# SajayR/TRIAD

Measured on AMD Instinct MI355X. Metric: tri-modal triples/sec (whole node) + loss parity, B=256 at 1/2/4/8 MI355X, higher is better.
Workload: dtype bf16

## Files before the change

include/triad_hip.h:

```cpp
#ifndef TRIAD_HIP_H
#define TRIAD_HIP_H

#include <hip/hip_runtime_api.h>

#ifdef __cplusplus
extern "C" {
#endif

#define TRIAD_EINVAL 1001

int triad_pairsim_nparts(int R_pad, int Bk);

int triad_pairsim_fwd(const void* Q, const void* K, int R, int R_pad, int Nq, int Bq, int Bk, int Nk_pad,
                      int Nk_eff, int D, const float* temp, float clamp_lo, int diag, int diag_off,
                      float* rowmax, int* argmax, double* nn_part, float* diagS, void* dS, long long CT,
                      double* st_part, const int* k_len, hipStream_t stream);

typedef struct triad_pairsim_problem {
  const void* Q;
  const void* K;
  int R, R_pad, Nq, Bq, Bk, Nk_pad, Nk_eff;
  const float* temp;
  float clamp_lo;
  int diag, diag_off;
// ... 128 lines not shown
                       hipStream_t stream);

int triad_grad_sumsq(const float* g, const void* chunks, int nchunks, double* out, hipStream_t stream);
int triad_adamw_step(float* p, const float* g, float* m, float* v, const void* chunks, int nchunks,
                     const float* pp, const float* scale, float beta1, float beta2, float omb1, float omb2,
                     float eps, const unsigned long long* shadow, hipStream_t stream);
int triad_gather_grads(const void* pieces, int npieces, float* g, int accumulate, hipStream_t stream);

int triad_gather_rows(const void* src, long long src_rows, const int* idx, int B, int M, int row_bytes, void* dst,
                      hipStream_t stream);

int triad_l2norm_rows(const void* x, int rows, int D, float eps, void* y, hipStream_t stream);

int triad_retrieval_maxmean_f32(const float* Q, const int* qlen, int Bq, int nq_pad, const float* K, const int* klen,
                                int Bk, int nk_pad, int D, float temp, float* sim, hipStream_t stream);

int triad_l2norm_rows_f32(const float* x, int rows, int D, float eps, float* y, hipStream_t stream);

long long triad_chgn_workspace_bytes(int B, int T, int C);
int triad_chgn_gelu_fwd(const void* x, int B, int T, int Tp, int C, const float* gamma, const float* beta,
                        float eps, float* mean, float* rstd, void* ws, void* y, hipStream_t stream);
int triad_chgn_gelu_bwd(const void* x, const void* dy, int B, int T, int Tp, int C, const float* gamma,
                        const float* beta, const float* mean, const float* rstd, void* ws, void* dx, float* dgamma,
                        float* dbeta, hipStream_t stream);

int triad_c0gn_fwd(const void* wave, long long Lp, const void* w0, int B, int T, int Tp, int C, const float* gamma,
                   const float* beta, float eps, float* mean, float* rstd, void* ws, void* out, void* y0out,
                   hipStream_t stream);

long long triad_conv0_dw_workspace_bytes(int B, int T, int C);
int triad_conv0_dw(const void* wave, long long Lp, const void* dy0, int B, int T, int Tp, int C, void* ws, float* dw0,
                   hipStream_t stream);

int triad_posconv(const void* x, const void* wt, const float* bias, void* y, int B, int T, int C, int groups,
                  int pad, hipStream_t stream);

long long triad_posconv_dw_part_bytes(int C, int groups, int splits);
int triad_posconv_dw(const void* x, const void* dy, int B, int T, int C, int groups, int pad, int splits, float* part,
                     hipStream_t stream);

int triad_attn_fwd(const void* q, long long q_sB, long long q_sN, const void* k, long long k_sB, long long k_sN,
                   const void* v, long long v_sB, long long v_sN, int B, int H, int N, int D, float scale, void* out,
                   long long out_sB, long long out_sN, float* lse, hipStream_t stream);
int triad_attn_bwd(const void* q, long long q_sB, long long q_sN, const void* k, long long k_sB, long long k_sN,
                   const void* v, long long v_sB, long long v_sN, const void* o, long long o_sB, long long o_sN,
                   const void* dout, long long do_sB, long long do_sN, const float* lse, int B, int H, int N, int D,
                   float scale, void* dq, long long dq_sB, long long dq_sN, void* dk, long long dk_sB,
                   long long dk_sN, void* dv, long long dv_sB, long long dv_sN, float* delta, hipStream_t stream);
int triad_attn_dropmask(int B, int H, int N, float p, unsigned seed, unsigned* wq, unsigned* wk, hipStream_t stream);
int triad_attn_fwd_dropout(const void* q, long long q_sB, long long q_sN, const void* k, long long k_sB,
                           long long k_sN, const void* v, long long v_sB, long long v_sN, int B, int H, int N, int D,
                           float scale, const unsigned* wq, float p, void* out, long long out_sB, long long out_sN,
                           float* lse, hipStream_t stream);
int triad_attn_bwd_dropout(const void* q, long long q_sB, long long q_sN, const void* k, long long k_sB,
                           long long k_sN, const void* v, long long v_sB, long long v_sN, const void* o,
                           long long o_sB, long long o_sN, const void* dout, long long do_sB, long long do_sN,
                           const float* lse, int B, int H, int N, int D, float scale, const unsigned* wq,
                           const unsigned* wk, float p, void* dq, long long dq_sB, long long dq_sN, void* dk,
                           long long dk_sB, long long dk_sN, void* dv, long long dv_sB, long long dv_sN, float* delta,
                           hipStream_t stream);

int triad_attn_long_dropmask(int B, int H, int N, float p, unsigned seed, unsigned* wq, unsigned* wk,
                             hipStream_t stream);
int triad_attn_long_fwd(const void* q, long long q_sB, long long q_sN, const void* k, long long k_sB, long long k_sN,
                        const void* v, long long v_sB, long long v_sN, int B, int H, int N, int D, float scale,
                        const unsigned* wq, float p, void* out, long long out_sB, long long out_sN, float* lse,
                        hipStream_t stream);
int triad_attn_long_bwd(const void* q, long long q_sB, long long q_sN, const void* k, long long k_sB, long long k_sN,
                        const void* v, long long v_sB, long long v_sN, const void* o, long long o_sB, long long o_sN,
                        const void* dout, long long do_sB, long long do_sN, const float* lse, int B, int H, int N,
                        int D, float scale, const unsigned* wq, const unsigned* wk, float p, void* dq, long long dq_sB,
                        long long dq_sN, void* dk, long long dk_sB, long long dk_sN, void* dv, long long dv_sB,
// ... 44 lines not shown
```

triad_amd/_lib.py:

```python
from __future__ import annotations

import ctypes as C
import os
import threading

_HERE = os.path.dirname(os.path.abspath(__file__))
DEFAULT_LIB = os.path.join(_HERE, "libtriad_hip.so")
LIB_PATH = os.environ.get("TRIAD_LIB_VARIANT", DEFAULT_LIB)

vp, i32, u32, i64, f32, f64 = C.c_void_p, C.c_int, C.c_uint, C.c_longlong, C.c_float, C.c_double

SIGNATURES = {
    "triad_pairsim_nparts": [i32, i32],
    "triad_pairsim_fwd": [vp, vp, i32, i32, i32, i32, i32, i32, i32, i32, vp, f32, i32, i32, vp, vp, vp, vp, vp,
                          i64, vp, vp, vp],
    "triad_pairsim_fwd_multi": [vp, i32, vp],
    "triad_pairsim_diag": [vp, i32, vp],
    "triad_clip_reduce": [vp, i32, i32, i32, i32, vp, vp, vp, vp],
    "triad_diag_smooth": [vp, i32, i32, i32, i32, f64, vp, vp, vp, vp],
    "triad_diag_sparsity": [vp, i32, i32, i32, i32, f32, f64, vp, vp, vp, vp],
    "triad_losshead": [vp, i32, i32, vp, vp, i32, f64, vp, i32, f64, f32, vp, vp, vp, vp],
    "triad_pairsim_dS": [vp, vp, i32, i32, i32, i32, i32, i32, i32, i32, vp, f32, i32, i32, vp, vp, vp, vp, vp,
                         vp, i64, vp, vp],
    "triad_split_pack": [vp, i32, i32, i32, i64, vp, vp, vp],
# ... 16 lines not shown
    "triad_gemm_bf16_bias_bf16": [vp, i64, i32, vp, i64, i32, i32, i32, i32, vp, vp, i64, vp],
    "triad_gemm_bf16_splitk": [vp, i64, i32, vp, i64, i32, i32, i32, i32, i32, vp, vp, vp, i32, vp],
    "triad_gemm_bf16_splitk_form": [vp, i64, i32, vp, i64, i32, i32, i32, i32, i32, vp, vp, vp, i32, i32, vp],
    "triad_wpack": [vp, i32, vp, vp],
    "triad_wpack2": [vp, i32, vp, vp, i32, vp, vp],
    "triad_projhead_fwd": [vp, i64, i32, i64, i64, i64, vp, vp, vp, vp, f32, vp, vp, vp, vp, vp, vp, vp, vp],
    "triad_similarity_maps": [vp, vp, i32, i32, i32, i32, vp, f32, vp, vp],
    "triad_rowpanel_count": [i64],
    "triad_projhead_ln_fwd": [vp, i64, i32, i64, i64, i64, vp, vp, vp, vp, f32, vp, vp, vp, vp, vp],
    "triad_rowgemm_bias": [vp, i64, i32, i64, vp, vp, vp, vp],
    "triad_projhead_ln_bwd": [vp, i64, vp, vp, vp, vp, vp, vp, vp, vp],
    "triad_ln_fwd": [vp, i32, vp, vp, f32, vp, vp, vp, vp],
    "triad_ln_bwd3": [vp, vp, vp, vp, vp, i32, vp, vp, i32, vp],
    "triad_sum_slabs": [vp, i32, i64, vp, i32, vp, vp],
    "triad_colsum_splits": [i64, i32],
    "triad_colsum": [vp, i64, i32, i64, vp, f32, i32, vp, vp],
    "triad_colsum_dma_splits": [i64, i32],
    "triad_colsum_dma": [vp, i64, i32, i64, vp, f32, i32, vp, vp],
    "triad_global_znorm": [vp, i64, f32, vp, vp, i32, vp],
    "triad_grad_sumsq": [vp, vp, i32, vp, vp],
    "triad_adamw_step": [vp, vp, vp, vp, vp, i32, vp, vp, f32, f32, f32, f32, f32, vp, vp],
    "triad_gather_grads": [vp, i32, vp, i32, vp],
    "triad_gather_rows": [vp, i64, vp, i32, i32, i32, vp, vp],
    "triad_l2norm_rows": [vp, i32, i32, f32, vp, vp],
    "triad_l2norm_rows_f32": [vp, i32, i32, f32, vp, vp],
    "triad_retrieval_maxmean_f32": [vp, vp, i32, i32, vp, vp, i32, i32, i32, f32, vp, vp],
    "triad_chgn_workspace_bytes": [i32, i32, i32],
    "triad_chgn_gelu_fwd": [vp, i32, i32, i32, i32, vp, vp, f32, vp, vp, vp, vp, vp],
    "triad_chgn_gelu_bwd": [vp, vp, i32, i32, i32, i32, vp, vp, vp, vp, vp, vp, vp, vp, vp],
    "triad_gemm_bf16_form": [vp, i64, i32, vp, i64, i32, i32, i32, i32, vp, vp, i64, i32, i32, vp],
    "triad_conv0_dw_workspace_bytes": [i32, i32, i32],
    "triad_conv0_dw": [vp, i64, vp, i32, i32, i32, i32, vp, vp, vp],
    "triad_c0gn_fwd": [vp, i64, vp, i32, i32, i32, i32, vp, vp, f32, vp, vp, vp, vp, vp, vp],
    "triad_posconv": [vp, vp, vp, vp, i32, i32, i32, i32, i32, vp],
    "triad_posconv_dw_part_bytes": [i32, i32, i32],
    "triad_posconv_dw": [vp, vp, i32, i32, i32, i32, i32, i32, vp, vp],
    "triad_rows_nt": [vp, i64, i32, i32, vp, i32, vp, vp],
    "triad_lora_update": [vp, i64, i32, i32, vp, vp, vp],
    "triad_dropaddln_fwd": [vp, vp, vp, vp, f32, i32, i32, f32, u32, vp, vp, vp, vp, vp],
    "triad_dropaddln_bwd_blocks": [i32],
    "triad_dropaddln_bwd": [vp, vp, vp, vp, vp, vp, vp, i32, i32, f32, u32, vp, vp, vp, vp],
    "triad_gelu_table_bytes": [],
    "triad_gelu_table": [vp, vp],
    "triad_geludrop_fwd": [vp, i64, f32, u32, vp, vp, vp],
    "triad_geludrop_bwd": [vp, vp, i64, f32, u32, vp, vp, vp],
    "triad_dropout_keep": [i64, f32, u32, vp, vp],
    "triad_addln_fwd": [vp, vp, vp, vp, vp, f32, i32, i32, vp, vp, i32, vp, vp, vp],
    "triad_addln_bwd": [vp, i32, vp, vp, vp, vp, vp, vp, i32, i32, vp, vp, vp],
    "triad_lora_tn_blocks": [i32],
    "triad_lora_tn": [vp, i64, i32, i32, vp, vp, vp, f32, vp, vp, vp],
    "triad_attn_dropmask": [i32, i32, i32, f32, u32, vp, vp, vp],
    "triad_attn_fwd_dropout": [vp, i64, i64, vp, i64, i64, vp, i64, i64, i32, i32, i32, i32, f32, vp, f32, vp, i64,
                               i64, vp, vp],
    "triad_attn_bwd_dropout": [vp, i64, i64, vp, i64, i64, vp, i64, i64, vp, i64, i64, vp, i64, i64, vp, i32, i32,
                               i32, i32, f32, vp, vp, f32, vp, i64, i64, vp, i64, i64, vp, i64, i64, vp, vp],
    "triad_attn_fwd": [vp, i64, i64, vp, i64, i64, vp, i64, i64, i32, i32, i32, i32, f32, vp, i64, i64, vp, vp],
    "triad_attn_bwd": [vp, i64, i64, vp, i64, i64, vp, i64, i64, vp, i64, i64, vp, i64, i64, vp, i32, i32, i32,
                       i32, f32, vp, i64, i64, vp, i64, i64, vp, i64, i64, vp, vp],
    "triad_attn_long_dropmask": [i32, i32, i32, f32, u32, vp, vp, vp],
    "triad_attn_long_fwd": [vp, i64, i64, vp, i64, i64, vp, i64, i64, i32, i32, i32, i32, f32, vp, f32, vp, i64, i64,
                            vp, vp],
    "triad_attn_long_bwd": [vp, i64, i64, vp, i64, i64, vp, i64, i64, vp, i64, i64, vp, i64, i64, vp, i32, i32, i32,
                            i32, f32, vp, vp, f32, vp, i64, i64, vp, i64, i64, vp, i64, i64, vp, vp],
    "triad_dense_nparts": [i64],
    "triad_dense_rowmax": [vp, i32, i32, i32, i32, i32, vp, vp, vp],
    "triad_nonneg_fwd": [vp, i64, f32, vp, vp],
    "triad_nonneg_bwd": [vp, i64, f32, f32, vp, vp, vp],
    "triad_sims_bwd_pack": [vp, vp, vp, vp, vp, i32, i32, i32, i32, i32, vp, vp, i64, vp, vp],
    "triad_sum_parts": [vp, i32, f64, vp, vp],
}
RESTYPES = {"triad_pairsim_nparts": C.c_int, "triad_chgn_workspace_bytes": C.c_longlong,
            "triad_conv0_dw_workspace_bytes": C.c_longlong, "triad_gelu_table_bytes": C.c_longlong,
            "triad_posconv_dw_part_bytes": C.c_longlong,
            "triad_lora_tn_blocks": C.c_int, "triad_dropaddln_bwd_blocks": C.c_int,
            "triad_colsum_splits": C.c_int, "triad_colsum_dma_splits": C.c_int, "triad_dense_nparts": C.c_int,
            "triad_rowpanel_count": C.c_int}

BACKBONE_ENTRY_POINTS = frozenset({
    "triad_chgn_gelu_fwd", "triad_chgn_gelu_bwd", "triad_gemm_bf16_form", "triad_conv0_dw", "triad_c0gn_fwd",
    "triad_posconv", "triad_posconv_dw", "triad_gemm_bf16_splitk", "triad_rows_nt", "triad_lora_update",
    "triad_dropaddln_fwd", "triad_dropaddln_bwd", "triad_gelu_table", "triad_geludrop_fwd", "triad_geludrop_bwd",
    "triad_dropout_keep", "triad_addln_fwd", "triad_addln_bwd", "triad_lora_tn", "triad_attn_dropmask",
    "triad_attn_fwd_dropout", "triad_attn_bwd_dropout", "triad_attn_fwd", "triad_attn_bwd",
    "triad_attn_long_dropmask", "triad_attn_long_fwd", "triad_attn_long_bwd"})


def hot_path_entry_points():
    return tuple(n for n in SIGNATURES if n not in RESTYPES and n not in BACKBONE_ENTRY_POINTS)



class PairsimProblem(C.Structure):
    _fields_ = [("Q", vp), ("K", vp), ("R", i32), ("R_pad", i32), ("Nq", i32), ("Bq", i32), ("Bk", i32),
                ("Nk_pad", i32), ("Nk_eff", i32), ("temp", vp), ("clamp_lo", f32), ("diag", i32), ("diag_off", i32),
                ("rowmax", vp), ("argmax", vp), ("nn_part", vp), ("diagS", vp), ("dS", vp), ("CT", i64),
                ("st_part", vp), ("k_tiles", vp)]


_lock = threading.Lock()
_lib = None


class TriadError(RuntimeError):
    pass


def load():
    global _lib
    with _lock:
        if _lib is None:
            if not os.path.exists(LIB_PATH):
                raise TriadError(f"{LIB_PATH} not found: build it with `python -m triad_amd.build` "
# ... 73 lines not shown
```

triad_amd/csrc/frontend.hip:

```cpp
#include "common.h"

namespace {

constexpr int CHUNK = 128;
constexpr int NT = 256;

struct V8 {
  float v[8];
};

__device__ __forceinline__ V8 load8(const bf16* p) {
  const bf16x8 r = *(const bf16x8*)p;
  V8 o;
#pragma unroll
  for (int i = 0; i < 8; ++i) o.v[i] = (float)r[i];
  return o;
}

__device__ __forceinline__ void store8(bf16* p, const V8& x) {
  bf16x8 r;
#pragma unroll
  for (int i = 0; i < 8; ++i) r[i] = (bf16)x.v[i];
  *(bf16x8*)p = r;
}
// ... 282 lines not shown
  for (int t = t0 + r0; t < t1; t += rows) {
    const V8 dv = load8(dy + ((size_t)b * Tp + t) * C + c0);
    const float* sp = smp + C0_S * (t - t0);
#pragma unroll
    for (int j = 0; j < C0_K; ++j) {
      const float sj = sp[j];
#pragma unroll
      for (int i = 0; i < 8; ++i) dw[i][j] = fmaf(dv.v[i], sj, dw[i][j]);
    }
  }
  float* dst = dwpart + ((size_t)b * nblk + blk) * C * C0_K;
#pragma unroll
  for (int j0 = 0; j0 < C0_K; j0 += 2) {
    __syncthreads();
#pragma unroll
    for (int i = 0; i < 8; ++i) {
      red[(threadIdx.x * 8 + i) * 2] = dw[i][j0];
      red[(threadIdx.x * 8 + i) * 2 + 1] = dw[i][j0 + 1];
    }
    __syncthreads();
    for (int c = threadIdx.x; c < C; c += NT) {
      const int g8 = c / 8, i = c % 8;
      float a0 = 0.f, a1 = 0.f;
      for (int r = 0; r < rows; ++r) {
        a0 += red[((r * tpr + g8) * 8 + i) * 2];
        a1 += red[((r * tpr + g8) * 8 + i) * 2 + 1];
      }
      dst[c * C0_K + j0] = a0;
      dst[c * C0_K + j0 + 1] = a1;
    }
  }
}

bool shape_ok(int B, int T, int C) {
  return B > 0 && T > 0 && C > 0 && C % 8 == 0 && NT % (C / 8) == 0;
}

}

extern "C" {

long long triad_chgn_workspace_bytes(int B, int T, int C) {
  const long long nchunk = (T + CHUNK - 1) / CHUNK;
  return (long long)B * nchunk * C * 8 + (long long)B * C * 8 + (long long)B * C * 16;
}

int triad_chgn_gelu_fwd(const void* x, int B, int T, int Tp, int C, const float* gamma, const float* beta,
                        float eps, float* mean, float* rstd, void* ws, void* y, hipStream_t stream) {
  if (!shape_ok(B, T, C) || Tp < T) return TRIAD_EINVAL;
  const int nchunk = (T + CHUNK - 1) / CHUNK;
  float2* part = (float2*)ws;
  hipLaunchKernelGGL(chgn_sums_kernel<0>, dim3(nchunk, B), dim3(NT), 0, stream, (const bf16*)x, nullptr, T, Tp, C,
                     nullptr, nullptr, nullptr, nullptr, part);
  hipLaunchKernelGGL(chgn_stats_kernel, dim3((C + 255) / 256, B), dim3(256), 0, stream, part, nchunk, T, C, eps,
                     mean, rstd);
  hipLaunchKernelGGL(chgn_apply_kernel<0>, dim3(nchunk, B), dim3(NT), 0, stream, (const bf16*)x, nullptr, T, Tp, C,
                     mean, rstd, gamma, beta, nullptr, (bf16*)y);
  TRIAD_CHECK_LAUNCH();
  return TRIAD_OK;
}

int triad_chgn_gelu_bwd(const void* x, const void* dy, int B, int T, int Tp, int C, const float* gamma,
                        const float* beta, const float* mean, const float* rstd, void* ws, void* dx, float* dgamma,
                        float* dbeta, hipStream_t stream) {
  if (!shape_ok(B, T, C) || Tp < T) return TRIAD_EINVAL;
  const int nchunk = (T + CHUNK - 1) / CHUNK;
// ... 10 lines not shown
  TRIAD_CHECK_LAUNCH();
  return TRIAD_OK;
}

int triad_c0gn_fwd(const void* wave, long long Lp, const void* w0, int B, int T, int Tp, int C, const float* gamma,
                   const float* beta, float eps, float* mean, float* rstd, void* ws, void* out, void* y0out,
                   hipStream_t stream) {
  if (!shape_ok(B, T, C) || Tp < T || Lp < (long long)C0_S * (Tp - 1) + C0_K) return TRIAD_EINVAL;
  const int nchunk = (T + CHUNK - 1) / CHUNK;
  float2* part = (float2*)ws;
  hipLaunchKernelGGL(c0gn_kernel<0>, dim3(nchunk, B), dim3(NT), 0, stream, (const bf16*)wave, Lp, (const bf16*)w0, T,
                     Tp, C, nullptr, nullptr, nullptr, nullptr, nullptr, nullptr, part);
  hipLaunchKernelGGL(chgn_stats_kernel, dim3((C + 255) / 256, B), dim3(256), 0, stream, part, nchunk, T, C, eps,
                     mean, rstd);
  hipLaunchKernelGGL(c0gn_kernel<1>, dim3(nchunk, B), dim3(NT), 0, stream, (const bf16*)wave, Lp, (const bf16*)w0, T,
                     Tp, C, mean, rstd, gamma, beta, (bf16*)out, (bf16*)y0out, nullptr);
  TRIAD_CHECK_LAUNCH();
  return TRIAD_OK;
}

long long triad_conv0_dw_workspace_bytes(int B, int T, int C) {
  return (long long)B * ((T + C0_DW_ROWS - 1) / C0_DW_ROWS) * C * C0_K * 4;
}

int triad_conv0_dw(const void* wave, long long Lp, const void* dy0, int B, int T, int Tp, int C, void* ws, float* dw0,
                   hipStream_t stream) {
  if (!shape_ok(B, T, C) || Tp < T || Lp < (long long)C0_S * (T - 1) + C0_K) return TRIAD_EINVAL;
  const int nblk = (T + C0_DW_ROWS - 1) / C0_DW_ROWS;
  hipLaunchKernelGGL(c0dw_kernel, dim3(nblk, B), dim3(NT), 0, stream, (const bf16*)wave, Lp, (const bf16*)dy0, T, Tp,
                     C, (float*)ws);
  TRIAD_CHECK_LAUNCH();
  return triad_sum_slabs((const float*)ws, B * nblk, (long long)C * C0_K, nullptr, 0, dw0, stream);
}
}
```

triad_amd/frontend.py:

```python
from __future__ import annotations

import types
from ctypes import c_void_p as C_void_p

import torch
import torch.nn as nn
import torch.nn.functional as F

from . import _lib
from ._lib import call, ptr, stream_ptr


def _compute_dtype(x):
    if x.is_cuda and torch.is_autocast_enabled("cuda"):
        return torch.get_autocast_dtype("cuda")
    return x.dtype


class _Conv1dGemm(torch.autograd.Function):

    @staticmethod
    def forward(ctx, x, w, bias, stride, need_dx, cd):
        B, T, C = x.shape
        O, Cw, k = w.shape
# ... 153 lines not shown

class _Conv0GNGelu(torch.autograd.Function):

    @staticmethod
    def forward(ctx, wave, w, gamma, beta, eps, Tp):
        B, L = wave.shape
        O = w.shape[0]
        T = (L - 10) // 5 + 1
        need = (Tp - 1) * 5 + 10
        xw = F.pad(wave.to(torch.bfloat16), (0, max(0, need - L))).contiguous()
        w0 = w.to(torch.bfloat16).reshape(O, 10).contiguous()
        g = gamma.detach().float().contiguous()
        b = beta.detach().float().contiguous()
        dev = wave.device
        mean = torch.empty(B, O, dtype=torch.float32, device=dev)
        rstd = torch.empty(B, O, dtype=torch.float32, device=dev)
        ws = torch.empty(int(call("triad_chgn_workspace_bytes", B, T, O)), dtype=torch.uint8, device=dev)
        out = torch.empty(B * Tp + 2, O, dtype=torch.bfloat16, device=dev)
        y0 = torch.empty(B * Tp, O, dtype=torch.bfloat16, device=dev)
        out[B * Tp:].zero_()
        call("triad_c0gn_fwd", ptr(xw), xw.shape[1], ptr(w0), B, T, Tp, O, ptr(g), ptr(b), float(eps), ptr(mean),
             ptr(rstd), ptr(ws), ptr(out), ptr(y0), stream_ptr(dev))
        ctx.save_for_backward(xw, y0, g, b, mean, rstd)
        ctx.meta = (B, T, Tp, w.shape, w.dtype, gamma.dtype, beta.dtype)
        return out

    @staticmethod
    def backward(ctx, dout):
        xw, y0, g, b, mean, rstd = ctx.saved_tensors
        B, T, Tp, wshape, wdt, gdt, bdt = ctx.meta
        O = y0.shape[1]
        dev = xw.device
        dy = dout[:B * Tp].to(torch.bfloat16).contiguous()
        ws = torch.empty(int(call("triad_chgn_workspace_bytes", B, T, O)), dtype=torch.uint8, device=dev)
        dy0 = torch.empty_like(y0)
        dg = torch.empty(O, dtype=torch.float32, device=dev)
        db = torch.empty(O, dtype=torch.float32, device=dev)
        call("triad_chgn_gelu_bwd", ptr(y0), ptr(dy), B, T, Tp, O, ptr(g), ptr(b), ptr(mean), ptr(rstd), ptr(ws),
             ptr(dy0), ptr(dg), ptr(db), stream_ptr(dev))
        dw = torch.empty(O, 10, dtype=torch.float32, device=dev)
        ws2 = torch.empty(int(call("triad_conv0_dw_workspace_bytes", B, T, O)), dtype=torch.uint8, device=dev)
        call("triad_conv0_dw", ptr(xw), xw.shape[1], ptr(dy0), B, T, Tp, O, ptr(ws2), ptr(dw), stream_ptr(dev))
        return None, dw.view(wshape).to(wdt), dg.to(gdt), db.to(bdt), None, None


class _FrameConvS2(torch.autograd.Function):

    @staticmethod
    def forward(ctx, x, w, B, Tp):
        Cin = x.shape[1]
        O, Cw, k = w.shape
        if Cw != Cin or k not in (2, 3) or Tp % 2 or x.shape[0] != B * Tp + 2:
            raise _lib.TriadError("frame conv: expects a [B*Tp + 2, C] buffer, even Tp, kernel 2 or 3")
        M = B * Tp // 2
        wr = w.to(torch.bfloat16).permute(0, 2, 1).reshape(O, k * Cin).contiguous()
        y = torch.empty(M + 2, O, dtype=torch.bfloat16, device=x.device)
        _gemm_rows(x, 0, 2 * Cin, M, k * Cin, wr, y, 0, O)
        y[M:].zero_()
        ctx.save_for_backward(x, w)
        ctx.meta = (B, Tp, w.dtype)
        return y

    @staticmethod
    def backward(ctx, dy):
        x, w = ctx.saved_tensors
        B, Tp, wdt = ctx.meta
        Cin = x.shape[1]
        O, _, k = w.shape
        M = B * Tp // 2
        dy = dy.to(torch.bfloat16).contiguous()
        wb = w.to(torch.bfloat16)
        wj = [wb[:, :, j] for j in range(k)]

        def weight_grad():
            dwr = _weight_grad_rows(dy, M, x, 2 * Cin, k * Cin)
# ... 119 lines not shown
        if ctx.needs_input_grad[0]:
            wtb = wb.view(G, Cg, Cg, K).flip(-1).permute(0, 2, 3, 1).reshape(G, Cg, K * Cg).contiguous()
            dx = torch.empty_like(dyb)
            call("triad_posconv", ptr(dyb), ptr(wtb), None, ptr(dx), B, T, C, G, K - 1 - pad, stream_ptr(xb.device))
            dx = dx.to(ctx.dtypes[0])
        if ctx.needs_input_grad[1] and C // G == 48:
            splits = max(1, min(B, 16))
            part = torch.empty(int(call("triad_posconv_dw_part_bytes", C, G, splits)) // 4, dtype=torch.float32,
                               device=dyb.device)
            call("triad_posconv_dw", ptr(xb), ptr(dyb), B, T, C, G, pad, splits, ptr(part), stream_ptr(dyb.device))
            cg = C // G
            dsum = torch.empty(part.numel() // splits, dtype=torch.float32, device=dyb.device)
            call("triad_sum_slabs", ptr(part), splits, dsum.numel(), None, 0, ptr(dsum), stream_ptr(dyb.device),
                 meta=dict(backbone=True))
            dw = dsum.view(G, K, cg, cg).permute(0, 2, 3, 1).reshape(C, cg, K)
            dw = dw.to(ctx.dtypes[1])
        elif ctx.needs_input_grad[1] and 128 % (C // G) == 0:
            dw = _posconv_dw_gemm(xb, dyb, G, pad, K).to(ctx.dtypes[1])
        elif ctx.needs_input_grad[1]:
            t_full = T + 2 * pad - K + 1
            dy_full = torch.zeros(B, t_full, C, dtype=torch.bfloat16, device=dyb.device)
            dy_full[:, :T] = dyb
            x4 = xb.transpose(1, 2).unsqueeze(2)
            dy4 = dy_full.transpose(1, 2).unsqueeze(2)
            dw = torch.ops.aten.convolution_backward(dy4, x4, wb.unsqueeze(2), None, [1, 1], [0, pad], [1, 1],
                                                     False, [0, 0], G, [False, True, False])[1]
            dw = dw.squeeze(2).to(ctx.dtypes[1])
        if ctx.has_bias and ctx.needs_input_grad[2]:
            from .ops import bias_grad
            db = bias_grad(dyb.view(B * T, C), torch.float32).to(ctx.dtypes[2])
        return dx, dw, db, None, None


def _posconv_dw_gemm(xb, dyb, G, pad, K):
    from ._lib import call, ptr, stream_ptr
    B, T, C = xb.shape
    CG = C // G
    P = 128 // CG
    Tp = T + K - 1
    rows = B * Tp
    Kd = (rows + 63) // 64 * 64
    dev = xb.device
    out = torch.empty(C, CG, K, dtype=torch.float32, device=dev)
    splits = 4
    slabs = torch.empty(splits * 128 * 128 * K, dtype=torch.float32, device=dev)
    blk = torch.empty(128, K * 128, dtype=torch.float32, device=dev)
    st = stream_ptr(dev)
    for c0 in range(0, C, 128):
        xp = torch.zeros(Kd + K, 128, dtype=torch.bfloat16, device=dev)
        xp[:rows].view(B, Tp, 128)[:, pad:pad + T] = xb[:, :, c0:c0 + 128]
        dyp = torch.zeros(Kd, 128, dtype=torch.bfloat16, device=dev)
        dyp[:rows].view(B, Tp, 128)[:, :T] = dyb[:, :, c0:c0 + 128]
        call("triad_gemm_bf16_splitk", ptr(dyp), 128, 0, ptr(xp), 128, 0, 128, K * 128, Kd, splits, None,
             ptr(slabs), ptr(blk), 0, st, meta=dict(backbone=True))
        v = blk.view(128, K, 128)
        for q in range(P):
            g0 = c0 + q * CG
            out[g0:g0 + CG] = v[q * CG:(q + 1) * CG, :, q * CG:(q + 1) * CG].permute(0, 2, 1)
    return out


def _hubert_pos_conv_forward(self, hidden_states):
    conv = self.conv
    if not hidden_states.is_cuda or getattr(self, "batch_norm", None) is not None \
            or _compute_dtype(hidden_states) != torch.bfloat16 or conv.kernel_size[0] != 128 \
            or getattr(self.padding, "num_pad_remove", 1) != 1:
        return self._triad_hf_forward(hidden_states)
    y = _PosConv.apply(hidden_states, conv.weight, conv.bias, conv.groups, conv.padding[0])
    return _hip_act(self.activation)(y)


class _SpecMask(torch.autograd.Function):

    @staticmethod
    def forward(ctx, h, m, emb):
        ctx.save_for_backward(m)
        ctx.emb_dtype = emb.dtype
        return torch.where(m[..., None], emb.to(h.dtype), h)

    @staticmethod
    def backward(ctx, g):
        (m,) = ctx.saved_tensors
        from .ops import bias_grad
        mm = m[..., None]
        gm = torch.where(mm, g, torch.zeros((), dtype=g.dtype, device=g.device))
        demb = bias_grad(gm.reshape(-1, g.shape[-1]).to(torch.bfloat16).contiguous(), torch.float32)
        return torch.where(mm, torch.zeros((), dtype=g.dtype, device=g.device), g), None, demb.to(ctx.emb_dtype)


def _spec_where(m, emb, h):
    if h.dtype == torch.bfloat16 and emb.requires_grad:
        return _SpecMask.apply(h, m, emb)
    return torch.where(m[..., None], emb.to(h.dtype), h)


def _hubert_mask_hidden_states(self, hidden_states, mask_time_indices=None, attention_mask=None):
    if not hidden_states.is_cuda:
        return self._triad_hf_mask(hidden_states, mask_time_indices=mask_time_indices, attention_mask=attention_mask)
    from transformers.models.hubert.modeling_hubert import _compute_mask_indices
    cfg = self.config
    if not getattr(cfg, "apply_spec_augment", True):
# ... 48 lines not shown
```

Measured before the change: 1971.

## Fuse conv0 GroupNorm-GELU backward with weight grad; native weight-norm for pos-conv

Replaces the two-pass conv0 backward (GN+GELU backward writing dy0, then a separate conv0 weight-grad pass) with a single fused kernel. It accumulates per-channel sums and waveform-weighted products directly, then finishes with small reduction kernels. It also adds native HIP kernels for the pos-conv weight-norm forward and backward, building both the forward and flipped weight images in one pass instead of going through the PyTorch parametrization. This removes the dy0 round trip and several generic ops, at the cost of more register pressure in the fused kernel and reassociated reductions that could shift loss parity slightly.

```diff
diff --git a/include/triad_hip.h b/include/triad_hip.h
--- a/include/triad_hip.h
+++ b/include/triad_hip.h
@@ -184,12 +184,24 @@
 int triad_conv0_dw(const void* wave, long long Lp, const void* dy0, int B, int T, int Tp, int C, void* ws, float* dw0,
                    hipStream_t stream);
 
+long long triad_c0gn_bwd_rows_per_block(void);
+long long triad_c0gn_bwd_workspace_bytes(int B, int T, int C);
+int triad_c0gn_bwd(const void* wave, long long Lp, const void* y0, const void* dy, int B, int T, int Tp, int C,
+                   const float* gamma, const float* mean, const float* rstd, const float* beta, void* ws, float* dw0,
+                   float* dgamma, float* dbeta, hipStream_t stream);
+
 int triad_posconv(const void* x, const void* wt, const float* bias, void* y, int B, int T, int C, int groups,
                   int pad, hipStream_t stream);
 
 long long triad_posconv_dw_part_bytes(int C, int groups, int splits);
 int triad_posconv_dw(const void* x, const void* dy, int B, int T, int C, int groups, int pad, int splits, float* part,
                      hipStream_t stream);
+
+long long triad_posconv_wn_workspace_bytes(int C, int groups);
+int triad_posconv_wn_fwd(const float* v, const float* g, int C, int groups, void* ws, float* norm, void* wt, void* wtb,
+                         hipStream_t stream);
+int triad_posconv_wn_bwd(const float* dws, const float* v, const float* g, const float* norm, int C, int groups,
+                         void* ws, float* dv, float* dg, hipStream_t stream);
 
 int triad_attn_fwd(const void* q, long long q_sB, long long q_sN, const void* k, long long k_sB, long long k_sN,
                    const void* v, long long v_sB, long long v_sN, int B, int H, int N, int D, float scale, void* out,
diff --git a/triad_amd/_lib.py b/triad_amd/_lib.py
--- a/triad_amd/_lib.py
+++ b/triad_amd/_lib.py
@@ -72,9 +72,15 @@
     "triad_conv0_dw_workspace_bytes": [i32, i32, i32],
     "triad_conv0_dw": [vp, i64, vp, i32, i32, i32, i32, vp, vp, vp],
     "triad_c0gn_fwd": [vp, i64, vp, i32, i32, i32, i32, vp, vp, f32, vp, vp, vp, vp, vp, vp],
+    "triad_c0gn_bwd_rows_per_block": [],
+    "triad_c0gn_bwd_workspace_bytes": [i32, i32, i32],
+    "triad_c0gn_bwd": [vp, i64, vp, vp, i32, i32, i32, i32, vp, vp, vp, vp, vp, vp, vp, vp, vp],
     "triad_posconv": [vp, vp, vp, vp, i32, i32, i32, i32, i32, vp],
     "triad_posconv_dw_part_bytes": [i32, i32, i32],
     "triad_posconv_dw": [vp, vp, i32, i32, i32, i32, i32, i32, vp, vp],
+    "triad_posconv_wn_workspace_bytes": [i32, i32],
+    "triad_posconv_wn_fwd": [vp, vp, i32, i32, vp, vp, vp, vp, vp],
+    "triad_posconv_wn_bwd": [vp, vp, vp, vp, i32, i32, vp, vp, vp, vp],
     "triad_rows_nt": [vp, i64, i32, i32, vp, i32, vp, vp],
     "triad_lora_update": [vp, i64, i32, i32, vp, vp, vp],
     "triad_dropaddln_fwd": [vp, vp, vp, vp, f32, i32, i32, f32, u32, vp, vp, vp, vp, vp],
@@ -111,13 +117,15 @@
 }
 RESTYPES = {"triad_pairsim_nparts": C.c_int, "triad_chgn_workspace_bytes": C.c_longlong,
             "triad_conv0_dw_workspace_bytes": C.c_longlong, "triad_gelu_table_bytes": C.c_longlong,
-            "triad_posconv_dw_part_bytes": C.c_longlong,
+            "triad_posconv_dw_part_bytes": C.c_longlong, "triad_c0gn_bwd_rows_per_block": C.c_longlong,
+            "triad_c0gn_bwd_workspace_bytes": C.c_longlong, "triad_posconv_wn_workspace_bytes": C.c_longlong,
             "triad_lora_tn_blocks": C.c_int, "triad_dropaddln_bwd_blocks": C.c_int,
             "triad_colsum_splits": C.c_int, "triad_colsum_dma_splits": C.c_int, "triad_dense_nparts": C.c_int,
             "triad_rowpanel_count": C.c_int}
 
 BACKBONE_ENTRY_POINTS = frozenset({
     "triad_chgn_gelu_fwd", "triad_chgn_gelu_bwd", "triad_gemm_bf16_form", "triad_conv0_dw", "triad_c0gn_fwd",
+    "triad_c0gn_bwd", "triad_posconv_wn_fwd", "triad_posconv_wn_bwd",
     "triad_posconv", "triad_posconv_dw", "triad_gemm_bf16_splitk", "triad_rows_nt", "triad_lora_update",
     "triad_dropaddln_fwd", "triad_dropaddln_bwd", "triad_gelu_table", "triad_geludrop_fwd", "triad_geludrop_bwd",
     "triad_dropout_keep", "triad_addln_fwd", "triad_addln_bwd", "triad_lora_tn", "triad_attn_dropmask",
diff --git a/triad_amd/csrc/frontend.hip b/triad_amd/csrc/frontend.hip
--- a/triad_amd/csrc/frontend.hip
+++ b/triad_amd/csrc/frontend.hip
@@ -338,6 +338,168 @@
   }
 }
 
+constexpr int C0B_ROWS = 1600;
+constexpr int C0B_NV = 2 + 2 * C0_K;
+constexpr int C0B_NO = 2 + C0_K;
+
+__device__ __forceinline__ void c0b_reduce2(float* red, const float (&a)[8], const float (&b)[8], int C, int tpr,
+                                            int rows, float* __restrict__ dst0, float* __restrict__ dst1) {
+  __syncthreads();
+#pragma unroll
+  for (int i = 0; i < 8; ++i) {
+    red[(threadIdx.x * 8 + i) * 2] = a[i];
+    red[(threadIdx.x * 8 + i) * 2 + 1] = b[i];
+  }
+  __syncthreads();
+  for (int c = threadIdx.x; c < C; c += NT) {
+    const int g8 = c / 8, i = c % 8;
+    float a0 = 0.f, a1 = 0.f;
+    for (int r = 0; r < rows; ++r) {
+      a0 += red[((r * tpr + g8) * 8 + i) * 2];
+      a1 += red[((r * tpr + g8) * 8 + i) * 2 + 1];
+    }
+    dst0[c] = a0;
+    dst1[c] = a1;
+  }
+}
+
+__global__ __launch_bounds__(NT) __attribute__((amdgpu_waves_per_eu(2))) void c0gn_bwd_kernel(
+    const bf16* __restrict__ wave, long long Lp, const bf16* __restrict__ y0, const bf16* __restrict__ dy, int T,
+    int Tp, int C, const float* __restrict__ mean, const float* __restrict__ rstd, const float* __restrict__ gamma,
+    const float* __restrict__ beta, float* __restrict__ part) {
+  static_assert(C0_S * C0B_ROWS + C0_K >= NT * 8 * 2, "the reduction buffer aliases the waveform span");
+  __shared__ __attribute__((aligned(16))) float smp[C0_S * C0B_ROWS + C0_K];
+  __shared__ __attribute__((aligned(16))) float cst[4][NT * 8];
+  float* red = smp;
+  const int b = blockIdx.y, blk = blockIdx.x, nblk = gridDim.x;
+  const int tpr = C / 8, rows = NT / tpr;
+  const int cg = threadIdx.x % tpr, r0 = threadIdx.x / tpr;
+  const int c0 = cg * 8;
+  const int t0 = blk * C0B_ROWS, t1 = min(T, t0 + C0B_ROWS);
+  const int nsmp = (t1 > t0) ? C0_S * (t1 - t0 - 1) + C0_K : 0;
+  for (int i = threadIdx.x; i < nsmp; i += NT) smp[i] = (float)wave[(long long)b * Lp + (long long)C0_S * t0 + i];
+  for (int c = threadIdx.x; c < C; c += NT) {
+    cst[0][c] = mean[(size_t)b * C + c];
+    cst[1][c] = rstd[(size_t)b * C + c];
+    cst[2][c] = gamma[c];
+    cst[3][c] = beta[c];
+  }
+  float s[8], q[8], P[C0_K][8], X[C0_K][8];
+#pragma unroll
+  for (int i = 0; i < 8; ++i) {
+    s[i] = 0.f;
+    q[i] = 0.f;
+#pragma unroll
+    for (int j = 0; j < C0_K; ++j) {
+      P[j][i] = 0.f;
+      X[j][i] = 0.f;
+    }
+  }
+  __syncthreads();
+  for (int t = t0 + r0; t < t1; t += rows) {
+    const size_t off = ((size_t)b * Tp + t) * C + c0;
+    const bf16x8 xr = *(const bf16x8*)(y0 + off);
+    const bf16x8 dr = *(const bf16x8*)(dy + off);
+    const float* sp = smp + C0_S * (t - t0);
+    float sv[C0_K];
+#pragma unroll
+    for (int j = 0; j < C0_K; ++j) sv[j] = sp[j];
+#pragma unroll
+    for (int h = 0; h < 2; ++h) {
+      int cc = c0 + 4 * h;
+      asm volatile("" : "+v"(cc));
+      const float4 mu4 = *(const float4*)&cst[0][cc], rs4 = *(const float4*)&cst[1][cc];
+      const float4 g4 = *(const float4*)&cst[2][cc], be4 = *(const float4*)&cst[3][cc];
+      const float mu[4] = {mu4.x, mu4.y, mu4.z, mu4.w}, rs[4] = {rs4.x, rs4.y, rs4.z, rs4.w};
+      const float g[4] = {g4.x, g4.y, g4.z, g4.w}, be[4] = {be4.x, be4.y, be4.z, be4.w};
+#pragma unroll
+      for (int k = 0; k < 4; ++k) {
+        const int i = 4 * h + k;
+        const float xh = ((float)xr[i] - mu[k]) * rs[k];
+        const float dz = (float)dr[i] * gelu_grad(fmaf(xh, g[k], be[k]));
+        s[i] += dz;
+        q[i] = fmaf(dz, xh, q[i]);
+#pragma unroll
+        for (int j = 0; j < C0_K; ++j) {
+          P[j][i] = fmaf(dz, sv[j], P[j][i]);
+          X[j][i] = fmaf(xh, sv[j], X[j][i]);
+        }
+      }
+    }
+  }
+  float* dst = part + ((size_t)b * nblk + blk) * C0B_NV * C;
+  c0b_reduce2(red, s, q, C, tpr, rows, dst, dst + C);
+#pragma unroll
+  for (int j = 0; j < C0_K; j += 2) {
+    c0b_reduce2(red, P[j], P[j + 1], C, tpr, rows, dst + (size_t)(2 + j) * C, dst + (size_t)(3 + j) * C);
+    c0b_reduce2(red, X[j], X[j + 1], C, tpr, rows, dst + (size_t)(2 + C0_K + j) * C,
+                dst + (size_t)(3 + C0_K + j) * C);
+  }
+}
+
+__global__ __launch_bounds__(NT) void c0b_s1_kernel(const bf16* __restrict__ wave, long long Lp, int T,
+                                                    double* __restrict__ s1) {
+  __shared__ double red[NT][C0_K];
+  const int b = blockIdx.x;
+  const bf16* w = wave + (long long)b * Lp;
+  double acc[C0_K];
+#pragma unroll
+  for (int j = 0; j < C0_K; ++j) acc[j] = 0.0;
+  for (int u = threadIdx.x; u <= T; u += NT) {
+#pragma unroll
+    for (int r = 0; r < C0_S; ++r) {
+      const double v = (double)(float)w[(long long)C0_S * u + r];
+      if (u < T) acc[r] += v;
+      if (u >= 1) acc[r + C0_S] += v;
+    }
+  }
+#pragma unroll
+  for (int j = 0; j < C0_K; ++j) red[threadIdx.x][j] = acc[j];
+  __syncthreads();
+  if (threadIdx.x < C0_K) {
+    double a = 0.0;
+    for (int i = 0; i < NT; ++i) a += red[i][threadIdx.x];
+    s1[(size_t)b * C0_K + threadIdx.x] = a;
+  }
+}
+
+__global__ void c0b_fin1_kernel(const float* __restrict__ part, const double* __restrict__ s1, int nblk, int T, int C,
+                                const float* __restrict__ gamma, const float* __restrict__ rstd,
+                                double* __restrict__ fin) {
+  const int b = blockIdx.y, c = blockIdx.x * blockDim.x + threadIdx.x;
+  if (c >= C) return;
+  double v[C0B_NV];
+#pragma unroll
+  for (int k = 0; k < C0B_NV; ++k) v[k] = 0.0;
+  for (int blk = 0; blk < nblk; ++blk) {
+    const float* src = part + ((size_t)b * nblk + blk) * C0B_NV * C + c;
+#pragma unroll
+    for (int k = 0; k < C0B_NV; ++k) v[k] += (double)src[(size_t)k * C];
+  }
+  const double gm = gamma[c], rs = rstd[(size_t)b * C + c];
+  const double cA = gm * v[0] / T, cB = gm * v[1] / T;
+  double* dst = fin + (size_t)b * C0B_NO * C + c;
+#pragma unroll
+  for (int j = 0; j < C0_K; ++j)
+    dst[(size_t)j * C] = rs * (gm * v[2 + j] - cA * s1[(size_t)b * C0_K + j] - cB * v[2 + C0_K + j]);
+  dst[(size_t)C0_K * C] = v[0];
+  dst[(size_t)(C0_K + 1) * C] = v[1];
+}
+
+__global__ void c0b_fin2_kernel(const double* __restrict__ fin, int B, int C, float* __restrict__ dw0,
+                                float* __restrict__ dgamma, float* __restrict__ dbeta) {
+  const int k = blockIdx.y, c = blockIdx.x * blockDim.x + threadIdx.x;
+  if (c >= C) return;
+  double a = 0.0;
+  for (int b = 0; b < B; ++b) a += fin[((size_t)b * C0B_NO + k) * C + c];
+  if (k < C0_K)
+    dw0[(size_t)c * C0_K + k] = (float)a;
+  else if (k == C0_K)
+    dbeta[c] = (float)a;
+  else
+    dgamma[c] = (float)a;
+}
+
 bool shape_ok(int B, int T, int C) {
   return B > 0 && T > 0 && C > 0 && C % 8 == 0 && NT % (C / 8) == 0;
 }
@@ -414,4 +576,30 @@
   TRIAD_CHECK_LAUNCH();
   return triad_sum_slabs((const float*)ws, B * nblk, (long long)C * C0_K, nullptr, 0, dw0, stream);
 }
-}
+
+long long triad_c0gn_bwd_rows_per_block(void) { return C0B_ROWS; }
+
+long long triad_c0gn_bwd_workspace_bytes(int B, int T, int C) {
+  const long long nblk = (T + C0B_ROWS - 1) / C0B_ROWS;
+  return (long long)B * C0B_NO * C * 8 + (long long)B * C0_K * 8 + (long long)B * nblk * C0B_NV * C * 4;
+}
+
+int triad_c0gn_bwd(const void* wave, long long Lp, const void* y0, const void* dy, int B, int T, int Tp, int C,
+                   const float* gamma, const float* mean, const float* rstd, const float* beta, void* ws, float* dw0,
+                   float* dgamma, float* dbeta, hipStream_t stream) {
+  if (!shape_ok(B, T, C) || Tp < T || Lp < (long long)C0_S * (T - 1) + C0_K) return TRIAD_EINVAL;
+  if (!wave || !y0 || !dy || !gamma || !mean || !rstd || !beta || !ws || !dw0 || !dgamma || !dbeta) return TRIAD_EINVAL;
+  const int nblk = (T + C0B_ROWS - 1) / C0B_ROWS;
+  double* fin = (double*)ws;
+  double* s1 = fin + (size_t)B * C0B_NO * C;
+  float* part = (float*)(s1 + (size_t)B * C0_K);
+  hipLaunchKernelGGL(c0b_s1_kernel, dim3(B), dim3(NT), 0, stream, (const bf16*)wave, Lp, T, s1);
+  hipLaunchKernelGGL(c0gn_bwd_kernel, dim3(nblk, B), dim3(NT), 0, stream, (const bf16*)wave, Lp, (const bf16*)y0,
+                     (const bf16*)dy, T, Tp, C, mean, rstd, gamma, beta, part);
+  hipLaunchKernelGGL(c0b_fin1_kernel, dim3((C + 255) / 256, B), dim3(256), 0, stream, part, s1, nblk, T, C, gamma, rstd,
+                     fin);
+  hipLaunchKernelGGL(c0b_fin2_kernel, dim3((C + 63) / 64, C0B_NO), dim3(64), 0, stream, fin, B, C, dw0, dgamma, dbeta);
+  TRIAD_CHECK_LAUNCH();
+  return TRIAD_OK;
+}
+}
diff --git a/triad_amd/csrc/posconv_wn.hip b/triad_amd/csrc/posconv_wn.hip
--- /dev/null
+++ b/triad_amd/csrc/posconv_wn.hip
@@ -0,0 +1,143 @@
+#include "common.h"
+
+namespace {
+
+constexpr int WN_K = 128, WN_CG = 48;
+constexpr int WN_NT = 256;
+constexpr int WN_SLAB = 256;
+constexpr int WN_LD = WN_CG + 1;
+
+__global__ __launch_bounds__(WN_NT) void wn_sumsq_kernel(const float* __restrict__ v, int rows,
+                                                         float* __restrict__ part) {
+  __shared__ float red[WN_K];
+  const int k = threadIdx.x % WN_K, h = threadIdx.x / WN_K;
+  const int r0 = blockIdx.x * WN_SLAB, r1 = min(rows, r0 + WN_SLAB);
+  float a = 0.f;
+  for (int r = r0 + h; r < r1; r += WN_NT / WN_K) {
+    const float x = v[(size_t)r * WN_K + k];
+    a = fmaf(x, x, a);
+  }
+  if (h == 1) red[k] = a;
+  __syncthreads();
+  if (h == 0) part[(size_t)blockIdx.x * WN_K + k] = a + red[k];
+}
+
+__global__ void wn_norm_kernel(const float* __restrict__ part, int nblk, float* __restrict__ norm,
+                               float* __restrict__ rnorm) {
+  const int k = threadIdx.x;
+  double a = 0.0;
+  for (int i = 0; i < nblk; ++i) a += (double)part[(size_t)i * WN_K + k];
+  const float n = (float)sqrt(a);
+  norm[k] = n;
+  rnorm[k] = 1.f / n;
+}
+
+__global__ __launch_bounds__(WN_NT) void wn_images_kernel(const float* __restrict__ v, const float* __restrict__ g,
+                                                          const float* __restrict__ rnorm, bf16* __restrict__ wt,
+                                                          bf16* __restrict__ wtb) {
+  __shared__ float tile[WN_K * WN_LD];
+  const int a = blockIdx.x, grp = blockIdx.y, flip = blockIdx.z;
+  for (int e = threadIdx.x; e < WN_CG * WN_K; e += WN_NT) {
+    const int r = e / WN_K, k = e % WN_K;
+    const int o = grp * WN_CG + (flip ? r : a), c = flip ? a : r;
+    tile[k * WN_LD + r] = g[k] * v[((size_t)o * WN_CG + c) * WN_K + k] * rnorm[k];
+  }
+  __syncthreads();
+  bf16* out = (flip ? wtb : wt) + ((size_t)grp * WN_CG + a) * WN_K * WN_CG;
+  for (int e = threadIdx.x; e < WN_K * WN_CG; e += WN_NT) {
+    const int j = e / WN_CG, r = e % WN_CG;
+    out[e] = (bf16)tile[(flip ? WN_K - 1 - j : j) * WN_LD + r];
+  }
+}
+
+__device__ __forceinline__ void wn_load_dw(const float* __restrict__ dws, int grp, int n, float* tile) {
+  for (int e = threadIdx.x; e < WN_K * WN_CG; e += WN_NT) {
+    const int j = e / WN_CG, c = e % WN_CG;
+    tile[j * WN_LD + c] = dws[(((size_t)grp * WN_K + j) * WN_CG + n) * WN_CG + c];
+  }
+}
+
+__global__ __launch_bounds__(WN_NT) void wn_bwd_dot_kernel(const float* __restrict__ dws, const float* __restrict__ v,
+                                                           float* __restrict__ dot) {
+  __shared__ float tile[WN_K * WN_LD];
+  __shared__ float red[WN_K];
+  const int n = blockIdx.x, grp = blockIdx.y, o = grp * WN_CG + n;
+  wn_load_dw(dws, grp, n, tile);
+  __syncthreads();
+  const int k = threadIdx.x % WN_K, h = threadIdx.x / WN_K;
+  float a = 0.f;
+  for (int c = h; c < WN_CG; c += WN_NT / WN_K) a = fmaf(tile[k * WN_LD + c], v[((size_t)o * WN_CG + c) * WN_K + k], a);
+  if (h == 1) red[k] = a;
+  __syncthreads();
+  if (h == 0) dot[(size_t)o * WN_K + k] = a + red[k];
+}
+
+__global__ __launch_bounds__(8 * WN_K) void wn_bwd_dg_kernel(const float* __restrict__ dot, int C, const float* __restrict__ norm,
+                                 float* __restrict__ dg) {
+  __shared__ double red[8][WN_K];
+  const int k = threadIdx.x % WN_K, h = threadIdx.x / WN_K;
+  double a = 0.0;
+  for (int o = h; o < C; o += 8) a += (double)dot[(size_t)o * WN_K + k];
+  red[h][k] = a;
+  __syncthreads();
+  if (h == 0) {
+    for (int i = 1; i < 8; ++i) a += red[i][k];
+    dg[k] = (float)(a / (double)norm[k]);
+  }
+}
+
+__global__ __launch_bounds__(WN_NT) void wn_bwd_dv_kernel(const float* __restrict__ dws, const float* __restrict__ v,
+                                                          const float* __restrict__ g, const float* __restrict__ norm,
+                                                          const float* __restrict__ dg, float* __restrict__ dv) {
+  __shared__ float tile[WN_K * WN_LD];
+  const int n = blockIdx.x, grp = blockIdx.y, o = grp * WN_CG + n;
+  wn_load_dw(dws, grp, n, tile);
+  __syncthreads();
+  const int k = threadIdx.x % WN_K, h = threadIdx.x / WN_K;
+  const float rn = 1.f / norm[k], s = g[k] * rn, t = dg[k] * rn;
+  for (int c = h; c < WN_CG; c += WN_NT / WN_K) {
+    const size_t i = ((size_t)o * WN_CG + c) * WN_K + k;
+    dv[i] = s * (tile[k * WN_LD + c] - v[i] * t);
+  }
+}
+
+bool wn_shape_ok(int C, int groups) { return C > 0 && groups > 0 && C % groups == 0 && C / groups == WN_CG; }
+
+}
+
+extern "C" {
+
+long long triad_posconv_wn_workspace_bytes(int C, int groups) {
+  if (!wn_shape_ok(C, groups)) return 0;
+  const long long rows = (long long)C * WN_CG;
+  const long long nblk = (rows + WN_SLAB - 1) / WN_SLAB;
+  const long long fwd = nblk * WN_K * 4 + WN_K * 4;
+  const long long bwd = (long long)C * WN_K * 4;
+  return fwd > bwd ? fwd : bwd;
+}
+
+int triad_posconv_wn_fwd(const float* v, const float* g, int C, int groups, void* ws, float* norm, void* wt, void* wtb,
+                         hipStream_t stream) {
+  if (!wn_shape_ok(C, groups) || !v || !g || !ws || !norm || !wt || !wtb) return TRIAD_EINVAL;
+  const int rows = C * WN_CG, nblk = (rows + WN_SLAB - 1) / WN_SLAB;
+  float* part = (float*)ws;
+  float* rnorm = part + (size_t)nblk * WN_K;
+  hipLaunchKernelGGL(wn_sumsq_kernel, dim3(nblk), dim3(WN_NT), 0, stream, v, rows, part);
+  hipLaunchKernelGGL(wn_norm_kernel, dim3(1), dim3(WN_K), 0, stream, part, nblk, norm, rnorm);
+  hipLaunchKernelGGL(wn_images_kernel, dim3(WN_CG, groups, 2), dim3(WN_NT), 0, stream, v, g, rnorm, (bf16*)wt,
+                     (bf16*)wtb);
+  TRIAD_CHECK_LAUNCH();
+  return TRIAD_OK;
+}
+
+int triad_posconv_wn_bwd(const float* dws, const float* v, const float* g, const float* norm, int C, int groups,
+                         void* ws, float* dv, float* dg, hipStream_t stream) {
+  if (!wn_shape_ok(C, groups) || !dws || !v || !g || !norm || !ws || !dv || !dg) return TRIAD_EINVAL;
+  float* dot = (float*)ws;
+  hipLaunchKernelGGL(wn_bwd_dot_kernel, dim3(WN_CG, groups), dim3(WN_NT), 0, stream, dws, v, dot);
+  hipLaunchKernelGGL(wn_bwd_dg_kernel, dim3(1), dim3(8 * WN_K), 0, stream, dot, C, norm, dg);
+  hipLaunchKernelGGL(wn_bwd_dv_kernel, dim3(WN_CG, groups), dim3(WN_NT), 0, stream, dws, v, g, norm, dg, dv);
+  TRIAD_CHECK_LAUNCH();
+  return TRIAD_OK;
+}
+}
diff --git a/triad_amd/frontend.py b/triad_amd/frontend.py
--- a/triad_amd/frontend.py
+++ b/triad_amd/frontend.py
@@ -209,15 +209,12 @@
         O = y0.shape[1]
         dev = xw.device
         dy = dout[:B * Tp].to(torch.bfloat16).contiguous()
-        ws = torch.empty(int(call("triad_chgn_workspace_bytes", B, T, O)), dtype=torch.uint8, device=dev)
-        dy0 = torch.empty_like(y0)
+        ws = torch.empty(int(call("triad_c0gn_bwd_workspace_bytes", B, T, O)), dtype=torch.uint8, device=dev)
         dg = torch.empty(O, dtype=torch.float32, device=dev)
         db = torch.empty(O, dtype=torch.float32, device=dev)
-        call("triad_chgn_gelu_bwd", ptr(y0), ptr(dy), B, T, Tp, O, ptr(g), ptr(b), ptr(mean), ptr(rstd), ptr(ws),
-             ptr(dy0), ptr(dg), ptr(db), stream_ptr(dev))
         dw = torch.empty(O, 10, dtype=torch.float32, device=dev)
-        ws2 = torch.empty(int(call("triad_conv0_dw_workspace_bytes", B, T, O)), dtype=torch.uint8, device=dev)
-        call("triad_conv0_dw", ptr(xw), xw.shape[1], ptr(dy0), B, T, Tp, O, ptr(ws2), ptr(dw), stream_ptr(dev))
+        call("triad_c0gn_bwd", ptr(xw), xw.shape[1], ptr(y0), ptr(dy), B, T, Tp, O, ptr(g), ptr(mean), ptr(rstd),
+             ptr(b), ptr(ws), ptr(dw), ptr(dg), ptr(db), stream_ptr(dev))
         return None, dw.view(wshape).to(wdt), dg.to(gdt), db.to(bdt), None, None
 
 
@@ -403,6 +400,87 @@
         return dx, dw, db, None, None
 
 
+class _PosConvWN(torch.autograd.Function):
+
+    @staticmethod
+    def forward(ctx, x, g, v, bias, groups, pad):
+        B, T, C = x.shape
+        dev = x.device
+        xb = x.to(torch.bfloat16).contiguous()
+        gc, vc = g.detach().contiguous(), v.detach().contiguous()
+        K = vc.shape[2]
+        ws = torch.empty(int(call("triad_posconv_wn_workspace_bytes", C, groups)), dtype=torch.uint8, device=dev)
+        norm = torch.empty(K, dtype=torch.float32, device=dev)
+        wt = torch.empty(groups, C // groups, K * (C // groups), dtype=torch.bfloat16, device=dev)
+        wtb = torch.empty_like(wt)
+        st = stream_ptr(dev)
+        call("triad_posconv_wn_fwd", ptr(vc), ptr(gc), C, groups, ptr(ws), ptr(norm), ptr(wt), ptr(wtb), st)
+        bf = None if bias is None else bias.detach().float().contiguous()
+        y = torch.empty_like(xb)
+        call("triad_posconv", ptr(xb), ptr(wt), ptr(bf), ptr(y), B, T, C, groups, pad, st)
+        ctx.save_for_backward(xb, wtb, gc, vc, norm)
+        ctx.groups, ctx.pad, ctx.has_bias = groups, pad, bias is not None
+        ctx.meta = (x.dtype, g.shape, None if bias is None else bias.dtype)
+        return y
+
+    @staticmethod
+    def backward(ctx, dy):
+        xb, wtb, gc, vc, norm = ctx.saved_tensors
+        B, T, C = xb.shape
+        G, pad, K = ctx.groups, ctx.pad, vc.shape[2]
+        xdt, gshape, bdt = ctx.meta
+        dev = xb.device
+        st = stream_ptr(dev)
+        dyb = dy.to(torch.bfloat16).contiguous()
+        dx = dg = dv = db = None
+        if ctx.needs_input_grad[0]:
+            dx = torch.empty_like(dyb)
+            call("triad_posconv", ptr(dyb), ptr(wtb), None, ptr(dx), B, T, C, G, K - 1 - pad, st)
+            dx = dx.to(xdt)
+        if ctx.needs_input_grad[1] or ctx.needs_input_grad[2]:
+            splits = max(1, min(B, 16))
+            part = torch.empty(int(call("triad_posconv_dw_part_bytes", C, G, splits)) // 4, dtype=torch.float32,
+                               device=dev)
+            call("triad_posconv_dw", ptr(xb), ptr(dyb), B, T, C, G, pad, splits, ptr(part), st)
+            dsum = torch.empty(part.numel() // splits, dtype=torch.float32, device=dev)
+            call("triad_sum_slabs", ptr(part), splits, dsum.numel(), None, 0, ptr(dsum), st, meta=dict(backbone=True))
+            ws = torch.empty(int(call("triad_posconv_wn_workspace_bytes", C, G)), dtype=torch.uint8, device=dev)
+            dv = torch.empty_like(vc)
+            dg = torch.empty(K, dtype=torch.float32, device=dev)
+            call("triad_posconv_wn_bwd", ptr(dsum), ptr(vc), ptr(gc), ptr(norm), C, G, ptr(ws), ptr(dv), ptr(dg), st)
+            dg = dg.view(gshape)
+        if ctx.has_bias and ctx.needs_input_grad[3]:
+            from .ops import bias_grad
+            db = bias_grad(dyb.view(B * T, C), torch.float32).to(bdt)
+        return dx, dg, dv, db, None, None
+
+
+def _weight_norm_originals(conv):
+    par = getattr(conv, "parametrizations", None)
+    if par is not None and "weight" in par:
+        plist = par["weight"]
+        if len(plist) == 1 and hasattr(plist, "original0") and hasattr(plist, "original1") \
+                and type(plist[0]).__name__ == "_WeightNorm":
+            return plist.original0, plist.original1, plist[0].dim
+        return None
+    if hasattr(conv, "weight_g") and hasattr(conv, "weight_v"):
+        for hook in conv._forward_pre_hooks.values():
+            if type(hook).__name__ == "WeightNorm" and getattr(hook, "name", None) == "weight":
+                return conv.weight_g, conv.weight_v, hook.dim
+    return None
+
+
+def _posconv_native_weight_norm(conv):
+    org = _weight_norm_originals(conv)
+    if org is None:
+        return None
+    g, v, dim = org
+    if dim != 2 or v.dim() != 3 or v.shape[1] != 48 or v.shape[2] != 128 or v.shape[0] != 48 * conv.groups \
+            or g.numel() != 128 or g.dtype != torch.float32 or v.dtype != torch.float32 or not v.is_cuda:
+        return None
+    return g, v
+
+
 def _posconv_dw_gemm(xb, dyb, G, pad, K):
     from ._lib import call, ptr, stream_ptr
     B, T, C = xb.shape
@@ -437,7 +515,11 @@
             or _compute_dtype(hidden_states) != torch.bfloat16 or conv.kernel_size[0] != 128 \
             or getattr(self.padding, "num_pad_remove", 1) != 1:
         return self._triad_hf_forward(hidden_states)
-    y = _PosConv.apply(hidden_states, conv.weight, conv.bias, conv.groups, conv.padding[0])
+    gv = _posconv_native_weight_norm(conv)
+    if gv is not None and hidden_states.shape[2] == gv[1].shape[0]:
+        y = _PosConvWN.apply(hidden_states, gv[0], gv[1], conv.bias, conv.groups, conv.padding[0])
+    else:
+        y = _PosConv.apply(hidden_states, conv.weight, conv.bias, conv.groups, conv.padding[0])
     return _hip_act(self.activation)(y)
 
 
```

Measured after the change: 1905. 3.3% lower.
